# tayloreisman16/LTE-GNU-Radio-Code

Measured on AMD Instinct MI355X. Metric: IQ Msamples/s through RX FFT+equalize, 2048-pt/144-CP; %HBM roofline; 1/2/4/8 GPU, higher is better.
Workload: dtype f32; 1 GPU; 2048-pt FFT / 144-CP / Kd=1200 / 16-QAM, 4369 frames x 240 symbols (1,048,560 symbols), AWGN loopback; frames_per_gpu=4369, symbols_per_gpu=1048560, outputs=equalised symbols + packed bits, parallelism=frame-shard x1, sync_search=screened

## Files before the change

### lte-gnu-radio-code_amd/csrc/capi_internal.hpp

```cpp
#pragma once
#include <hip/hip_runtime.h>

#include <algorithm>
#include <cmath>
#include <complex>
#include <cstdarg>
#include <cstdio>
#include <cstdlib>
#include <cstring>
#include <initializer_list>
#include <new>
#include <string>
#include <vector>

#include "../../include/ofdm_mi355x.h"
#ifdef OFDM_EXPERIMENTS
#include "../../tools/experiments/ofdm_experiments.h"
#endif
#include "ofdm_launch.hpp"

using namespace ofdm;

#pragma GCC visibility push(hidden)
int fail(int code, const char* fmt, ...);
// ... 11 lines not shown
        if (e_ != hipSuccess) return fail(OFDM_ERR_HIP, "%s: %s", #expr, hipGetErrorString(e_));   \
    } while (0)

struct ofdm_rx {
    ofdm_rx_cfg cfg{};
    hipStream_t stream = nullptr;
    hipStream_t stream2 = nullptr;
    hipEvent_t ev_up = nullptr, ev_s1 = nullptr;
    RxDev dev{};
    cf* d_tw = nullptr;
    cf* d_zc = nullptr;
    int count = 0;
    int corr_obs = -1;
    double tsr[3] = {0, 0, 0};
    cf* d_in = nullptr;
    int64_t in_cap = 0;
    cf* d_edf = nullptr;
    cf* d_pack = nullptr;
    int* pin_tsr = nullptr;
    int* pin_tsr_dev = nullptr;
    static constexpr size_t PIN_IN_BYTES = size_t(1024) << 10, PIN_OUT_BYTES = size_t(256) << 10;
    cf* pin_in = nullptr;
    cf* pin_in_dev = nullptr;
    cf* pin_out = nullptr;
    cf* pin_out_dev = nullptr;
    int* s_tsr = nullptr;
    cf* s_H = nullptr;
    cf* s_htime = nullptr;
    cf* s_esf = nullptr;
    cf* s_eqg = nullptr;
    cf* s_gain = nullptr;
    cf* s_ysc = nullptr;
    float* d_trial_m = nullptr;
    int* d_trial_d = nullptr;
    static constexpr int TRIAL_CAP = 1024;
    double* d_partial = nullptr;
    int64_t cap_frames = 0;
    int* f_tsr = nullptr;
    cf* f_H = nullptr;
    cf* f_gain = nullptr;
    cf* f_htime = nullptr;
    int win_pre = 0, win_post = 0;
    float* f_tail = nullptr;
    int64_t tail_frames = -1;
    int avg_n = 0;
    float* f_spread = nullptr;
    int64_t spread_frames = -1;
    cf* a_part_d = nullptr;
    cf* a_part_a0 = nullptr;
    float* a_part_q = nullptr;
    int* a_part_n = nullptr;
    int64_t cap_avg_frames = 0, cap_avg_items = 0;
    double* f_seg_partial = nullptr;
    int64_t cap_seg_partial = 0;
    int n_pilots = 0;
    int* p_idx = nullptr;
    float* p_k = nullptr;
    uint16_t* p_src = nullptr;
    cf pilot_conj = cf{1.f, 0.f};
    float p_kbar = 0.f, p_inv_skk = 0.f;
    cf* f_usum = nullptr;
    int64_t cap_usum = 0;
    int64_t last_frames = 0;
    double* c_part_e = nullptr;
    long long* c_part_n = nullptr;
    int64_t cap_csi_items = 0;
    float2* c_tab = nullptr;
    float* c_a = nullptr;
    int64_t cap_csi_tab = 0;
    float2* m_tab = nullptr;
    int64_t cap_mrc_tab = 0;
    double* m_sigma2 = nullptr;
    int64_t cap_mrc_units = 0;
    float* t_ws = nullptr;
    int64_t cap_turbo = 0;
    uint8_t* tb_ws = nullptr;
    int64_t cap_tb = 0;
    int max_trials = 0;
    int scan_block = 0;
    cf* d_scan_g = nullptr;
    int* d_seg_state = nullptr;
    unsigned* d_work = nullptr;
    bool use_queue = true;
    bool seg_armed = false;
    int variant = 0;
    unsigned* d_stamps = nullptr;
    bool profiling = false;
    static constexpr int PROF_RING = 32;
    hipEvent_t ev[3 * PROF_RING] = {};
    int64_t prof_calls = 0;
};

struct ofdm_fo {
    ofdm_fo_cfg cfg{};
    hipStream_t stream = nullptr;
    RxDev dev{};
    cf* d_tw = nullptr;
    cf* d_zc = nullptr;
    cf* d_rot = nullptr;
    int count = 0;
    int cor_obs = -1;
    int dmax_tmp_ind = -1;
    double tsr[OFDM_FO_MAX_SYNC][3] = {};
    cf* d_in = nullptr;
    int64_t in_cap = 0;
    int* t_tsr = nullptr;
    cf* t_H = nullptr;
    cf* t_htime = nullptr;
    cf* t_esf = nullptr;
    cf* t_gain = nullptr;
    cf* t_edf = nullptr;
    cf* d_code = nullptr;
    cf* t_edfd = nullptr;
    int n_spread = 0;
    cf* s_eqg = nullptr;
    cf* s_ysc = nullptr;
    float* d_trial_m = nullptr;
    int* d_trial_d = nullptr;
    static constexpr int TRIAL_WIN = 256;
    int64_t cap_frames = 0;
    int64_t cap_table = 0;
    float* b_tm = nullptr;
    int* b_td = nullptr;
    int* b_tsr = nullptr;
    int* b_fo = nullptr;
    cf* b_gain = nullptr;
    cf* b_edf = nullptr;
};

struct ofdm_trk {
    ofdm_trk_cfg cfg{};
    hipStream_t stream = nullptr;
    RxDev dev{};
    cf* d_tw = nullptr;
    cf* d_zc = nullptr;
    cf* d_in = nullptr;
    int64_t in_cap = 0;
    int64_t n_in = 0;
    int* t_tsr = nullptr;
    cf* t_H = nullptr;
    cf* t_imp = nullptr;
    cf* t_esf = nullptr;
    cf* t_gain = nullptr;
    cf* t_edf = nullptr;
    cf* s_ysc = nullptr;
    float* d_trial_m = nullptr;
    int* d_trial_d = nullptr;
    static constexpr int TRIAL_CAP = 4096;
};

struct ofdm_tx {
    ofdm_tx_cfg cfg{};
    hipStream_t stream = nullptr;
    TxDev dev{};
    cf* d_tw = nullptr;
    cf* d_zc = nullptr;
    cf* d_sync_time = nullptr;
    int* d_pilots = nullptr;
    int n_pilots = 0;
    cf pilot_value = cf{1.f, 0.f};
    uint8_t* tb_ws = nullptr;
    int64_t cap_tb = 0;
};

namespace {

// ... 203 lines not shown
```

### lte-gnu-radio-code_amd/csrc/capi_rx.hip

```cpp
#include "capi_internal.hpp"

namespace {
constexpr int SEG_STATE_0[2] = {0x7fffffff, 0};
}

extern "C" {

int ofdm_rx_destroy(ofdm_rx* h) {
    if (!h) return OFDM_OK;
    (void)hipSetDevice(h->cfg.device);
    if (h->pin_tsr) (void)hipHostFree(h->pin_tsr);
    if (h->pin_in) (void)hipHostFree(h->pin_in);
    if (h->pin_out) (void)hipHostFree(h->pin_out);
    free_dev(&h->tb_ws, &h->d_pack, &h->d_tw, &h->d_zc, &h->d_in, &h->d_edf, &h->s_tsr, &h->s_H, &h->s_htime, &h->s_esf, &h->s_eqg, &h->s_gain,
             &h->s_ysc, &h->d_trial_m, &h->d_trial_d, &h->d_partial, &h->f_tsr, &h->f_H, &h->f_gain, &h->f_htime, &h->d_scan_g,
             &h->d_seg_state, &h->d_work, &h->f_seg_partial, &h->p_idx, &h->p_k, &h->p_src, &h->f_usum, &h->t_ws, &h->c_part_e,
             &h->c_part_n, &h->c_tab, &h->c_a, &h->m_tab, &h->m_sigma2, &h->f_tail, &h->f_spread, &h->a_part_d, &h->a_part_a0, &h->a_part_q, &h->a_part_n);
    for (hipEvent_t e : h->ev)
        if (e) (void)hipEventDestroy(e);
    if (h->ev_up) (void)hipEventDestroy(h->ev_up);
    if (h->ev_s1) (void)hipEventDestroy(h->ev_s1);
    if (h->stream2) (void)hipStreamDestroy(h->stream2);
    if (h->stream) (void)hipStreamDestroy(h->stream);
    delete h;
// ... 41 lines not shown
    h->d_stamps = static_cast<unsigned*>(d_stamps);
    return OFDM_OK;
}
#endif

int ofdm_rx_set_sync_search(ofdm_rx* h, int32_t exhaustive) {
    if (!h) return fail(OFDM_ERR_INVALID, "null handle");
    h->scan_block = exhaustive ? 0 : rx_sync_scan_block(h->dev);
    if (h->scan_block > 0 && !h->d_scan_g) h->scan_block = 0;
    return h->scan_block > 0 ? 1 : 0;
}

int ofdm_rx_set_max_trials(ofdm_rx* h, int32_t max_trials) {
    if (!h || max_trials < 0) return fail(OFDM_ERR_INVALID, "bad argument");
    h->max_trials = max_trials;
    return OFDM_OK;
}

int ofdm_rx_create(const ofdm_rx_cfg* c, ofdm_rx** out) {
    if (!c || !out) return fail(OFDM_ERR_INVALID, "ofdm_rx_create: null argument");
    *out = nullptr;
    if (int bad = check_nfft(c->nfft)) return bad;
    if (c->cp_len < 0 || c->cp_len >= c->nfft) return fail(OFDM_ERR_INVALID, "cp_len=%d out of range", c->cp_len);
    if (int bad = check_bins(c->nfft, c->num_synch_bins, c->num_data_bins)) return bad;
    if (int bad = check_pattern(c->synch_S, c->synch_D, c->num_ofdm_symb)) return bad;
    if (c->modulation != 1 && c->modulation != 2 && c->modulation != 4 && c->modulation != 6)
        return fail(OFDM_ERR_INVALID, "modulation must be 1, 2, 4 or 6 bits per symbol");
    if (c->compat == OFDM_COMPAT_RXOFDM && c->cp_len < 2)
        return fail(OFDM_ERR_INVALID, "gr-RXOFDM search stride is cp_len-1: cp_len must be >= 2");
    if (c->compat != OFDM_COMPAT_UTSA && c->compat != OFDM_COMPAT_RXOFDM) return fail(OFDM_ERR_INVALID, "bad compat");

    HIP_TRY(hipSetDevice(c->device));
    ofdm_rx* h = new (std::nothrow) ofdm_rx();
    if (!h) return fail(OFDM_ERR_NOMEM, "out of host memory");
    h->cfg = *c;
    const int N = c->nfft, Ks = c->num_synch_bins, Kd = c->num_data_bins, S = c->synch_S;
    const int MM = S * Ks;
    RxDev& d = h->dev;
    const int root = fill_rxdev(*c, d);

    int rc = OFDM_OK;
    hipError_t e = hipStreamCreateWithFlags(&h->stream, hipStreamNonBlocking);
    if (e != hipSuccess) {
        rc = fail(OFDM_ERR_HIP, "hipStreamCreate: %s", hipGetErrorString(e));
    }
    if (rc == OFDM_OK && (hipStreamCreateWithFlags(&h->stream2, hipStreamNonBlocking) != hipSuccess ||
                          hipEventCreateWithFlags(&h->ev_up, hipEventDisableTiming) != hipSuccess ||
                          hipEventCreateWithFlags(&h->ev_s1, hipEventDisableTiming) != hipSuccess))
        rc = fail(OFDM_ERR_HIP, "second stream / events of the stream block");
    auto zc = make_zc(MM, root, c->compat == OFDM_COMPAT_UTSA ? MM : Ks);
    const size_t rows = size_t(c->num_ofdm_symb);
    if (rc == OFDM_OK) rc = upload_rx_tables(d, &h->d_tw, &h->d_zc, zc);
    if (rc == OFDM_OK) rc = alloc_zeroed(&h->d_edf, rows * Kd);
    if (rc == OFDM_OK) rc = dev_alloc(&h->d_pack, rows * Kd);
    if (rc == OFDM_OK && (hipHostMalloc(reinterpret_cast<void**>(&h->pin_tsr), 4 * sizeof(int), hipHostMallocMapped) != hipSuccess ||
                          hipHostMalloc(reinterpret_cast<void**>(&h->pin_in), ofdm_rx::PIN_IN_BYTES, hipHostMallocMapped) != hipSuccess ||
                          hipHostMalloc(reinterpret_cast<void**>(&h->pin_out), ofdm_rx::PIN_OUT_BYTES, hipHostMallocMapped) != hipSuccess ||
                          hipHostGetDevicePointer(reinterpret_cast<void**>(&h->pin_tsr_dev), h->pin_tsr, 0) != hipSuccess ||
                          hipHostGetDevicePointer(reinterpret_cast<void**>(&h->pin_in_dev), h->pin_in, 0) != hipSuccess ||
                          hipHostGetDevicePointer(reinterpret_cast<void**>(&h->pin_out_dev), h->pin_out, 0) != hipSuccess))
        rc = fail(OFDM_ERR_NOMEM, "pinned host allocation failed");
    if (rc == OFDM_OK) rc = alloc_zeroed(&h->s_tsr, 4);
    if (rc == OFDM_OK) rc = alloc_zeroed(&h->s_H, size_t(2) * N);
    if (rc == OFDM_OK) rc = alloc_zeroed(&h->s_htime, size_t(2) * N);
    if (rc == OFDM_OK) rc = alloc_zeroed(&h->s_esf, size_t(2) * MM);
    if (rc == OFDM_OK) rc = alloc_zeroed(&h->s_eqg, size_t(Ks));
    if (rc == OFDM_OK) rc = alloc_zeroed(&h->s_gain, size_t(Kd));
    if (rc == OFDM_OK) rc = dev_alloc(&h->s_ysc, size_t(MM));
    if (rc == OFDM_OK) rc = dev_alloc(&h->d_trial_m, size_t(ofdm_rx::TRIAL_CAP));
    if (rc == OFDM_OK) rc = dev_alloc(&h->d_trial_d, size_t(ofdm_rx::TRIAL_CAP));
    if (rc == OFDM_OK) rc = dev_alloc(&h->d_partial, size_t(DEMAP_PARTIALS));
    if (rc == OFDM_OK) rc = alloc_zeroed(&h->d_work, 2, "work queue init failed");
    h->scan_block = rx_sync_scan_block(d);
    if (rc == OFDM_OK && h->scan_block > 0) {
        rc = upload(&h->d_scan_g, make_scan_table(N, Ks, zc), "scan table upload failed");
        if (rc == OFDM_OK) rc = upload(&h->d_seg_state, SEG_STATE_0, 2, "segment state upload failed");
        h->seg_armed = rc == OFDM_OK;
    }
    if (rc != OFDM_OK) return create_failed(h, rc, ofdm_rx_destroy);
#ifdef OFDM_EXPERIMENTS
    if (const char* ev = std::getenv("OFDM_EXP_VARIANT")) h->variant = std::atoi(ev);
#endif
    if (const char* q = std::getenv("OFDM_MI355X_DEMOD_QUEUE")) h->use_queue = std::atoi(q) != 0;
    *out = h;
    return OFDM_OK;
}

int ofdm_rx_reserve(ofdm_rx* h, int64_t n_frames) {
    if (!h || n_frames < 0) return fail(OFDM_ERR_INVALID, "ofdm_rx_reserve: bad argument");
    if (n_frames <= h->cap_frames) return OFDM_OK;
    h->last_frames = 0;
    h->tail_frames = -1;
    h->spread_frames = -1;
    return regrow(h, {{&h->cap_frames, n_frames}}, ws_buf(&h->f_tsr, size_t(n_frames) * 4),
                  ws_buf(&h->f_H, size_t(n_frames) * h->dev.nfft), ws_buf(&h->f_gain, size_t(n_frames) * h->dev.Kd),
                  ws_buf(&h->f_htime, size_t(n_frames) * h->dev.nfft), ws_buf(&h->f_tail, size_t(n_frames)),
                  ws_buf(&h->f_spread, size_t(n_frames)));
}

int64_t ofdm_rx_demod_frames(ofdm_rx* h, const float* d_iq, int64_t n_frames, int64_t frame_stride,
                             int64_t frame_len, float* d_eq, uint8_t* d_bits, int32_t bits_mode, int32_t* d_tsr,
                             void* stream) {
    if (!h || !d_iq || n_frames < 0 || frame_len < 0 || frame_stride < frame_len)
        return fail(OFDM_ERR_INVALID, "ofdm_rx_demod_frames: bad argument");
    const RxDev& d = h->dev;
    const int SD = d.S + d.D;
    const int64_t n_unique = frame_len / d.L;
    const int64_t n_pat = n_unique / SD;
    const int64_t n_dsym = n_pat * d.D;
    const char* bad = demod_bad_args(d, n_frames, n_dsym, d_bits, bits_mode);
    if (*bad) return fail(OFDM_ERR_INVALID, "%s", bad);
    if (n_frames == 0) return n_dsym;
    HIP_TRY(hipSetDevice(h->cfg.device));
    if (n_frames > h->cap_frames) {
        int rc = ofdm_rx_reserve(h, n_frames);
        if (rc != OFDM_OK) return rc;
    }
    hipStream_t s = pick_stream(h, stream);

    SyncArgs sa{};
    sa.iq = reinterpret_cast<const cf*>(d_iq);
    sa.frame_stride = frame_stride;
    sa.frame_len = frame_len;
    sa.n_frames = int(n_frames);
    sa.mode = 0;
    sa.p_begin = 0;
    sa.p_count = h->max_trials;
    sa.force_accept = 0;
    sa.tsr = h->f_tsr;
    sa.H = h->f_H;
    sa.H_for_gain = nullptr;
    sa.gain = h->f_gain;
    sa.htime = nullptr;
    sa.scan_block = h->scan_block;
    sa.scan_g = h->d_scan_g;
#ifdef OFDM_EXPERIMENTS
    sa.stamps = h->d_stamps;
#endif
    hipEvent_t* pev = h->ev + 3 * (h->prof_calls % ofdm_rx::PROF_RING);
    if (h->profiling) HIP_TRY(hipEventRecord(pev[0], s));
    HIP_TRY(launch_rx_sync(d, sa, s));
    h->last_frames = n_frames;
    h->tail_frames = -1;
    h->spread_frames = -1;
    if (h->avg_n != 0) {
        const int rc = chan_average_in_place(h, sa.iq, n_frames, frame_stride, frame_len, s);
        if (rc != OFDM_OK) return rc;
    }
    if (h->win_post > 0) {
        ChanWinArgs wa{};
        wa.H_in = h->f_H;
        wa.tsr = h->f_tsr;
        wa.n_rows = n_frames;
        wa.pre = h->win_pre;
        wa.post = h->win_post;
        wa.H_out = h->f_H;
        wa.gain = h->f_gain;
        wa.tail = h->f_tail;
        HIP_TRY(launch_chan_window(d, wa, s));
        h->tail_frames = n_frames;
    }
    if (h->profiling) HIP_TRY(hipEventRecord(pev[1], s));

    if (n_dsym > 0 && (d_eq || d_bits)) {
        DemodArgs da{};
        da.iq = sa.iq;
        da.frame_stride = frame_stride;
        da.frame_len = frame_len;
        da.n_frames = int(n_frames);
        da.tsr = h->f_tsr;
        da.gain = h->f_gain;
        da.eq = reinterpret_cast<cf*>(d_eq);
        da.bits = d_bits;
        da.bits_mode = bits_mode;
        da.mod = d.bps;
        da.n_dsym = int(n_dsym);
        da.spc = 0;
        da.chunks_per_frame = 0;
        da.row_stride_pat = d.D;
        da.rows_per_frame = int(n_dsym);
        da.zero_skipped = 1;
        da.variant = h->variant;
        da.stamps = h->d_stamps;
        da.work = h->use_queue ? h->d_work : nullptr;
        HIP_TRY(launch_rx_demod(d, da, s));
    }
    if (h->profiling) {
        HIP_TRY(hipEventRecord(pev[2], s));
        h->prof_calls += 1;
    }
    if (d_tsr) HIP_TRY(hipMemcpyAsync(d_tsr, h->f_tsr, size_t(n_frames) * 4 * sizeof(int), hipMemcpyDeviceToDevice, s));
    return n_dsym;
}

int ofdm_rx_get_frame_state(ofdm_rx* h, int64_t frame, float* h_chan_freq, float* h_gain, float* h_chan_time) {
    if (!h || frame < 0 || frame >= h->cap_frames) return fail(OFDM_ERR_INVALID, "ofdm_rx_get_frame_state: bad frame");
    HIP_TRY(hipSetDevice(h->cfg.device));
    HIP_TRY(hipDeviceSynchronize());
    const int N = h->dev.nfft, Kd = h->dev.Kd;
    if (h_chan_freq) HIP_TRY(hipMemcpy(h_chan_freq, h->f_H + frame * N, size_t(N) * sizeof(cf), hipMemcpyDeviceToHost));
    if (h_gain) HIP_TRY(hipMemcpy(h_gain, h->f_gain + frame * Kd, size_t(Kd) * sizeof(cf), hipMemcpyDeviceToHost));
    if (h_chan_time) {
        HIP_TRY(launch_rx_chan_time(h->dev, h->f_H + frame * N, h->f_htime + frame * N, 1, h->stream));
        HIP_TRY(hipStreamSynchronize(h->stream));
        HIP_TRY(hipMemcpy(h_chan_time, h->f_htime + frame * N, size_t(N) * sizeof(cf), hipMemcpyDeviceToHost));
    }
    return OFDM_OK;
}

int ofdm_rx_get_state(ofdm_rx* h, int32_t row, float* h_chan_freq, float* h_chan_time, float* h_synch_freq,
                      float* h_eq_gain, float* h_data_freq) {
    if (!h || row < 0 || row > 1) return fail(OFDM_ERR_INVALID, "ofdm_rx_get_state: bad argument");
    HIP_TRY(hipSetDevice(h->cfg.device));
    HIP_TRY(hipStreamSynchronize(h->stream));
    const int N = h->dev.nfft, Kd = h->dev.Kd, Ks = h->dev.Ks, MM = h->dev.MM;
    if (h_chan_freq) HIP_TRY(hipMemcpy(h_chan_freq, h->s_H + size_t(row) * N, size_t(N) * sizeof(cf), hipMemcpyDeviceToHost));
    if (h_chan_time) HIP_TRY(hipMemcpy(h_chan_time, h->s_htime + size_t(row) * N, size_t(N) * sizeof(cf), hipMemcpyDeviceToHost));
    if (h_synch_freq) HIP_TRY(hipMemcpy(h_synch_freq, h->s_esf + size_t(row) * MM, size_t(MM) * sizeof(cf), hipMemcpyDeviceToHost));
    if (h_eq_gain) HIP_TRY(hipMemcpy(h_eq_gain, h->s_eqg, size_t(Ks) * sizeof(cf), hipMemcpyDeviceToHost));
    if (h_data_freq)
        HIP_TRY(hipMemcpy(h_data_freq, h->d_edf, size_t(h->cfg.num_ofdm_symb) * Kd * sizeof(cf), hipMemcpyDeviceToHost));
    return OFDM_OK;
}

}
namespace {
hipError_t upload_in(ofdm_rx* h, const float* h_in, int64_t from, int64_t to, hipStream_t s) {
    return hipMemcpyAsync(h->d_in + from, h_in + 2 * from, size_t(to - from) * sizeof(cf), hipMemcpyHostToDevice, s);
}

int deleted_rows(int rows, int SD) {
    int n_del = 0;
    for (int r = 3; r < rows; r += SD) ++n_del;
    return n_del;
}

SyncArgs final_args(const ofdm_rx* h, const cf* iq, int64_t n_in, int row) {
    const RxDev& d = h->dev;
    SyncArgs fa{};
    fa.iq = iq;
    fa.frame_stride = n_in;
    fa.frame_len = n_in;
    fa.n_frames = 1;
    fa.mode = 0;
    fa.tsr = h->s_tsr;
    fa.H = h->s_H + size_t(row) * d.nfft;
    fa.H_for_gain = (row == 0) ? nullptr : h->s_H;
    fa.gain = h->s_gain;
    fa.htime = h->s_htime + size_t(row) * d.nfft;
    fa.esf = h->s_esf + size_t(row) * d.MM;
    fa.eqg = h->s_eqg;
    fa.yscratch = h->s_ysc;
    return fa;
}

void add_segments(SyncArgs& fa, const ofdm_rx* h, int64_t p0, int64_t p_valid) {
    fa.p_begin = int(p0);
    fa.p_count = int(p_valid);
    fa.keep_on_miss = 1;
    fa.scan_block = h->scan_block;
    fa.scan_g = h->d_scan_g;
    fa.seg_len = h->scan_block;
    fa.n_seg = int((p_valid - p0 + fa.seg_len - 1) / fa.seg_len);
    fa.seg_state = h->d_seg_state;
}

DemodArgs loop_b_args(const ofdm_rx* h, const cf* iq, int64_t n_in, int64_t n_dsym) {
// ... 267 lines not shown
```

### lte-gnu-radio-code_amd/csrc/ofdm_launch.hpp

```cpp
#pragma once
#include <hip/hip_runtime.h>
#include <stdint.h>
#include <algorithm>
#include <vector>
#include "ofdm_device.hpp"

namespace ofdm {

template <class... Kernel>
inline hipError_t load_kernels(Kernel*... kernels) {
    hipFuncAttributes fa;
    hipError_t e = hipSuccess;
    ((e = e == hipSuccess ? hipFuncGetAttributes(&fa, reinterpret_cast<const void*>(kernels)) : e), ...);
    return e;
}

struct DemodArgs {
    const cf* iq;
    int64_t frame_stride;
    int64_t frame_len;
    int n_frames;
    const int* tsr;
    const cf* gain;
    cf* eq;
    uint8_t* bits;
    int bits_mode;
    int mod;
    int n_dsym;
    int spc;
    int chunks_per_frame;
    int row_stride_pat;
    int rows_per_frame;
    int zero_skipped;
    int variant;
    unsigned* stamps;
    const cf* rot;
    int host_guard;
    unsigned* work;
    int units_per_frame;
    const int* rot_idx;
};

struct SyncArgs {
    const cf* iq;
    int64_t frame_stride;
    int64_t frame_len;
    int n_frames;
    int mode;
    int p_begin;
    int p_count;
    int force_accept;
    int* tsr;
    cf* H;
    const cf* H_for_gain;
    cf* gain;
    cf* htime;
    cf* esf;
    cf* eqg;
    cf* yscratch;
    float* trial_m;
    int* trial_d;
    const cf* rot;
    int n_rot;
    int off_delta;
    int host_valid;
    int gain_lag_set;
    int gain_lag;
    int force_dhat_p1;
    int scan_block;
    const cf* scan_g;
    unsigned* stamps;
    int keep_on_miss;
    int* tsr_host;
    int n_seg;
    int seg_len;
    int* seg_state;
    int seg_base;
    int seg_launch;
    int seg_final;
};

struct FoDecideArgs {
    const float* trial_m;
    const int* trial_d;
    int n_frames;
    int n_rot;
    int p_count;
    int rows;
    int err_index;
    int* status;
    int* tsr_out;
    int* fo_idx;
    int* u_tsr;
};

constexpr int SYNC_STAGE_SEGS = 64;

struct DemapArgs {
    const cf* sym;
    int64_t n;
    int mod;
    uint8_t* hard;
    float* soft0;
    float* soft1;
    double* partial;
};
constexpr int DEMAP_PARTIALS = 256;

constexpr int SEG_SLICE = 2048;
inline int64_t seg_slices(int64_t seg_len) { return (seg_len + SEG_SLICE - 1) / SEG_SLICE; }
enum : int { SEG_OUT_SOFT0 = 1, SEG_OUT_SOFT1 = 2, SEG_OUT_LLR = 4 };
struct SegDemapArgs {
    const cf* sym;
    int64_t n_seg, seg_len, seg_stride;
    int64_t n_slices;
    int mod;
    float* soft0;
    float* soft1;
    float* llr;
    double* sigma;
    double* partial;
};

// ... 420 lines not shown
```

### lte-gnu-radio-code_amd/csrc/rx_demod.hpp

```cpp
#pragma once
#include <algorithm>
#include <atomic>
#include <cstdlib>
#include <type_traits>

#include "ofdm_launch.hpp"
#include "demap_hard.hpp"

#ifndef OFDM_NS_T128
#define OFDM_NS_T128 2
#endif
#ifndef OFDM_MINW_T128
#define OFDM_MINW_T128 3
#endif
#ifndef OFDM_FLAGS_T128
#define OFDM_FLAGS_T128 0u
#endif
#ifndef OFDM_FLAGS_T256
#define OFDM_FLAGS_T256 0u
#endif
#ifndef OFDM_LANE_TW
#define OFDM_LANE_TW 1
#endif
#ifndef OFDM_SCATTER_HOIST
// ... 79 lines not shown
    int* const qslot = reinterpret_cast<int*>(smem + DG::Q_OFF);
    int64_t chunk = blockIdx.x;
    if (a.work) {
        if (tid == 0) *qslot = int(atomicAdd(a.work, 1u));
        __syncthreads();
        chunk = *qslot;
    }
    for (; chunk < n_chunks;) {
    const int frame = int(chunk / a.chunks_per_frame);
    const int cidx = int(chunk % a.chunks_per_frame);
    const int trips = (a.n_dsym + NS - 1) / NS;
    const int ds0 = int(int64_t(cidx) * trips / a.chunks_per_frame) * NS;
    const int ds1 = min(int(int64_t(cidx + 1) * trips / a.chunks_per_frame) * NS, a.n_dsym);
    constexpr bool active = true;

    const int Kd = KD > 0 ? KD : rx.Kd, L = rx.L, S = rx.S, D = rx.D;
    const int tsr0 = a.tsr[frame * 4 + 0];
    const bool frame_on = (HG || UNITS) ? (a.tsr[frame * 4 + 3] != 0) : true;
    const int src_frame = UNITS ? frame / a.units_per_frame : frame;
    const cf* frame_iq = a.iq + int64_t(L2IN ? (blockIdx.x & 7) : src_frame) * a.frame_stride;
    const cf* rotp = (UNITS && ROT) ? a.rot + int64_t(max(a.rot_idx[src_frame], 0)) * N : a.rot;

    const cf* gain = a.gain + int64_t(frame) * Kd;
    cf* glds = smem + DG::G_OFF;
    const cf* gsrc = GLDS ? glds : gain;
    if constexpr (GLDS) {
        for (int i = 2 * tid; i < Kd; i += 2 * DG::WG) *reinterpret_cast<float4*>(glds + i) = *reinterpret_cast<const float4*>(gain + i);
    }
    float4 greg[GREG ? Q : 1][2];
    if constexpr (GREG) {
#pragma unroll
        for (int q = 0; q < Q; ++q)
#pragma unroll
            for (int hx = 0; hx < 2; ++hx) {
                const int idx = 4 * T * q + 256 * (t >> 6) + 128 * hx + 2 * (t & 63);
                greg[q][hx] = idx < Kd ? *reinterpret_cast<const float4*>(gain + idx) : float4{0.f, 0.f, 0.f, 0.f};
            }
    }

    const float sqrt_kd = sqrtf(float(Kd));
    const int n_iter = (ds1 - ds0 + NS - 1) / NS;
    struct Sym {
        bool valid, compute;
        int64_t start, orow;
    };
    auto sym_of = [&](int it) {
        Sym sy;
        const int itr = it;
        const int ds = ds0 + itr * NS + slot;
        sy.valid = active && it < n_iter && ds < ds1;
        const int p = ds / D, n_ = ds - p * D;
        const int64_t pat_ptr = int64_t(tsr0) + int64_t(S) * L * (int64_t(p) * (S + D) + 1);
        sy.compute = sy.valid && (HG ? frame_on : (pat_ptr + N - 1 <= a.frame_len)) && (!UNITS || frame_on);
        sy.start = pat_ptr + int64_t(L) * n_;
        sy.orow = int64_t(frame) * a.rows_per_frame + (p * a.row_stride_pat + n_);
        return sy;
    };
    cf v[P];
    auto load_sym = [&](const Sym& sy) {
        if (sy.compute && sy.start >= 0 && sy.start + N <= a.frame_len) {
            const cf* src = frame_iq + sy.start + t;
#pragma unroll
            for (int n0 = 0; n0 < P; ++n0) v[n0] = NTL ? __builtin_nontemporal_load(src + T * n0) : src[T * n0];
            if constexpr (ROT) {
#pragma unroll
                for (int n0 = 0; n0 < P; ++n0) v[n0] = cmul(v[n0], rotp[t + T * n0]);
            }
        } else {
            const int64_t before = -sy.start, left = a.frame_len - sy.start;
            const int lo = int(before < 0 ? 0 : (before < N ? before : N)), hi = int(left < 0 ? 0 : (left < N ? left : N));
            const bool any = sy.compute && hi > lo;
            int tq = t;
            asm volatile("" : "+v"(tq));
#pragma unroll
            for (int n0 = 0; n0 < P; ++n0) {
                const int e = tq + T * n0;
                const cf x = any ? frame_iq[sy.start + min(max(e, lo), hi - 1)] : cf{0.f, 0.f};
                v[n0] = (any && e >= lo && e < hi) ? x : cf{0.f, 0.f};
                if constexpr (ROT) v[n0] = cmul(v[n0], rotp[tq + T * n0]);
            }
        }
    };

    Sym cur = sym_of(0);
    if constexpr (PIPE) load_sym(cur);
    if constexpr (WL) wg_barrier();
    for (int it = 0; it < n_iter; ++it) {
        if constexpr (!PIPE) {
            cur = sym_of(it);
            load_sym(cur);
        }
        const bool sym_valid = cur.valid, compute = cur.compute;
        const int64_t orow = cur.orow;
        stamp(0);
        if constexpr (STAMP) asm volatile("s_waitcnt vmcnt(0)" ::: "memory");
        stamp(1);
        if constexpr (STAMP) {
            fft_pass0_store<N>(v, lds, tw, t);
            wg_barrier();
            stamp(2);
            if constexpr (PL::THREE) {
                fft_pass1_load<N>(v, lds, t);
                wg_barrier();
                fft_pass1_store<N>(v, lds, w1tab, t);
                wg_barrier();
            }
            stamp(3);
            fft_last_load<N>(v, lds, t);
            fft_last_dft<N>(v);
        } else {
            wg_fft<N, decltype(tw), WL>(v, lds, tw, w1tab, t);
        }
        slot_sync<WL>();

        int Kd_ = Kd;
#if !OFDM_SCATTER_HOIST
        asm volatile("" : "+s"(Kd_));
#endif
        const int hk = Kd_ >> 1;
        const int off_neg = hk - N, off_pos = hk - 1;
        float pse = 0.f;
#pragma unroll
        for (int j = 0; j < PL::C; ++j) {
#pragma unroll
            for (int kl = 0; kl < PL::RL; ++kl) {
#if OFDM_SCATTER_SKIP
                if constexpr (T >= 64) {
                    const int base = T * j + PL::NC * kl;
                    if (base > hk && base + T - 1 < N - hk) continue;
                }
#endif
                const int k = (t + T * j) + PL::NC * kl;
#if OFDM_SCATTER_SKIP
                if constexpr (T >= 64) {
                    const int base = T * j + PL::NC * kl;
                    const bool all_pos = base >= 1 && base + T - 1 <= hk, all_neg = base >= N - hk && hk < N / 2;
                    if (all_pos || all_neg) {
                        lds[k + (all_neg ? off_neg : off_pos)] = v[out_slot<N>(j, kl)];
                        if constexpr (PSE) pse += cnorm2(v[out_slot<N>(j, kl)]);
                        continue;
                    }
                }
#endif
                int i = k + ((k >= N - hk) ? off_neg : off_pos);
                if (j == 0 && kl == 0) i = (k == 0) ? N : i;
                lds[i] = v[out_slot<N>(j, kl)];
                if constexpr (PSE) pse += (unsigned(i) < unsigned(Kd_)) ? cnorm2(v[out_slot<N>(j, kl)]) : 0.f;
            }
        }
        if (Kd_ == N) {
#pragma unroll
            for (int j = 0; j < PL::C; ++j) {
#pragma unroll
                for (int kl = 0; kl < PL::RL; ++kl)
                    if ((t + T * j) + PL::NC * kl == N / 2) {
                        lds[N - 1] = v[out_slot<N>(j, kl)];
                        if constexpr (PSE) pse += cnorm2(v[out_slot<N>(j, kl)]);
                    }
            }
        }
        if constexpr (PSE) {
            pse = lanes_sum<T>(pse);
            if constexpr (T > 64) {
                if ((t & 63) == 0) red[t >> 6] = pse;
            }
        }
// ... 84 lines not shown
                                g = greg[q][hx];
                            else
                                g = *reinterpret_cast<const float4*>(g_lane + cofs);
                            const float4 av = *reinterpret_cast<const float4*>(l_lane + cofs);
                            cf z[2] = {cf{av.x, av.y} * scale, cf{av.z, av.w} * scale};
                            cmul2(z[0], cf{g.x, g.y}, z[1], cf{g.z, g.w});
                            if (eq_row) {
                                typedef float f4 __attribute__((ext_vector_type(4)));
                                const f4 ov = f4{z[0].x, z[0].y, z[1].x, z[1].y};
                                cf* const blk = eq_row + cofs;
#ifdef OFDM_EXPERIMENTS
                                constexpr unsigned SPOL = (FLAGS >> 12) & 3u;
                                if constexpr (SPOL == 1) {
                                    asm volatile("global_store_dwordx4 %0, %1, %2 sc1" ::"v"(eq_off), "v"(ov), "s"(blk) : "memory");
                                } else if constexpr (SPOL == 2) {
                                    asm volatile("global_store_dwordx4 %0, %1, %2 sc0 sc1" ::"v"(eq_off), "v"(ov), "s"(blk) : "memory");
                                } else if constexpr (SPOL == 3) {
                                    asm volatile("global_store_dwordx4 %0, %1, %2 sc0 sc1 nt" ::"v"(eq_off), "v"(ov), "s"(blk) : "memory");
                                } else
#endif
                                if constexpr (NT) {
                                    asm volatile("global_store_dwordx4 %0, %1, %2 nt" ::"v"(eq_off), "v"(ov), "s"(blk) : "memory");
                                } else {
                                    asm volatile("global_store_dwordx4 %0, %1, %2" ::"v"(eq_off), "v"(ov), "s"(blk) : "memory");
                                }
                            }
                            if constexpr (BMODE == 1) wp[hx] = pack2<MOD, ASMB>(z);
                            if constexpr (BMODE == 2) store_bits_pair_unpacked<MOD>(bits_row + cofs * MOD, unsigned(lane_e), z);
                        };
                        if (base + 128 <= Kd_) {
                            pair();
                        } else if (base < Kd_) {
                            if (base + 2 * lnm < Kd_) pair();
                        }
                    }
                    if constexpr (BMODE == 1) {
                        const bool odd = (ln & 1) != 0;
                        const unsigned recv = unsigned(__builtin_amdgcn_mov_dpp(int(odd ? wp[0] : wp[1]), 0xB1, 0xF, 0xF, false));
                        const unsigned w4 = odd ? ((recv << (2 * MOD)) | wp[1]) : ((wp[0] << (2 * MOD)) | recv);
                        const int ge = lane_e + (odd ? 126 : 0);
                        uint8_t* const brow = bits_row + (4 * T * q / 4) * (MOD / 2);
                        if (b0 + 256 <= Kd_) {
                            store_packed4<MOD>(brow, unsigned(ge), w4);
                        } else if (4 * T * q + ((KD > 0) ? opaque_lane(ge) : ge) < Kd_) {
                            store_packed4<MOD>(brow, unsigned(ge), w4);
                        }
                    }
                }
            }
        } else {
#pragma unroll
            for (int q = 0; q < Q; ++q) {
                const int idx = 4 * (t + T * q);
                if (idx < Kd_) {
                    const bool four = idx + 2 < Kd_;
                    const float4 g01 = *reinterpret_cast<const float4*>(gsrc + idx);
                    const float4 g23 = (GLDS || four) ? *reinterpret_cast<const float4*>(gsrc + idx + 2) : float4{0.f, 0.f, 0.f, 0.f};
                    const float4 a01 = *reinterpret_cast<const float4*>(lds + idx);
                    const float4 a23 = *reinterpret_cast<const float4*>(lds + idx + 2);
                    cf z[4] = {cf{a01.x, a01.y} * scale, cf{a01.z, a01.w} * scale, cf{a23.x, a23.y} * scale,
                               cf{a23.z, a23.w} * scale};
                    cmul3(z[0], cf{g01.x, g01.y}, z[1], cf{g01.z, g01.w}, z[2], cf{g23.x, g23.y});
                    z[3] = cmul(z[3], cf{g23.z, g23.w});
                    if (a.eq) {
                        float4* o = reinterpret_cast<float4*>(a.eq + orow * Kd_ + idx);
                        const float4 o0 = float4{z[0].x, z[0].y, z[1].x, z[1].y}, o1 = float4{z[2].x, z[2].y, z[3].x, z[3].y};
                        if constexpr (NT) {
                            typedef float f4 __attribute__((ext_vector_type(4)));
                            f4* on = reinterpret_cast<f4*>(o);
                            __builtin_nontemporal_store(f4{o0.x, o0.y, o0.z, o0.w}, on);
                            if (four) __builtin_nontemporal_store(f4{o1.x, o1.y, o1.z, o1.w}, on + 1);
                        } else {
                            o[0] = o0;
                            if (four) o[1] = o1;
                        }
                    }
                    if constexpr (BMODE != 0) store_bits<MOD, BMODE, ASMB>(a.bits, orow * Kd_ + idx, z, four ? 4 : 2);
                }
            }
        }
        stamp(6);
        slot_sync<WL>();
        stamp(7);
    }
    if (!a.work) break;
    __syncthreads();
    if (tid == 0) *qslot = int(atomicAdd(a.work, 1u));
    __syncthreads();
    chunk = *qslot;
    }
    if (a.work) {
        if (tid == 0 && atomicAdd(a.work + 1, 1u) == gridDim.x - 1) {
            atomicExch(a.work, 0u);
            atomicExch(a.work + 1, 0u);
        }
    }
    if constexpr (STAMP) {
        if ((tid & 63) == 0 && a.stamps) {
            unsigned* o = a.stamps + (int64_t(blockIdx.x) * (DG::WG / 64) + (tid >> 6)) * 8;
#pragma unroll
            for (int i = 0; i < 8; ++i) o[i] = acc[i];
        }
    }
}

template <int N, int KD>
hipError_t launch_rx_demod_batch(const RxDev& rx, DemodArgs a, unsigned grid, size_t lds, int bmode, hipStream_t s) {
    using DG = DemodGeom<N>;
    constexpr int MW = (Plan<N>::T == 128) ? OFDM_MINW_T128 : 3;
    constexpr unsigned FL = (Plan<N>::T == 128) ? OFDM_FLAGS_T128 : (Plan<N>::T == 256) ? OFDM_FLAGS_T256 : 0u;
#define OFDM_LD(M, B)                                                                                                        \
    do {                                                                                                                     \
        static std::atomic<int> announced{65536};                \
        if (int(lds) > announced.load(std::memory_order_relaxed)) {                                                          \
            hipError_t e = hipFuncSetAttribute(reinterpret_cast<const void*>(&rx_demod_kernel<N, M, B, MW, FL, KD>),         \
                                               hipFuncAttributeMaxDynamicSharedMemorySize, int(lds));                       \
            if (e != hipSuccess) return e;                                                                                   \
            announced.store(int(lds), std::memory_order_relaxed);                                                            \
        }                                                                                                                    \
        hipLaunchKernelGGL((rx_demod_kernel<N, M, B, MW, FL, KD>), dim3(grid), dim3(DG::WG), lds, s, rx, a);                 \
    } while (0)
    if (N < 1024) a.work = nullptr;
    if (a.work) {
        static int per_cu = 0, n_cu = 0;
        if (per_cu == 0) {
            int nb = 0, dev = 0;
            hipDeviceProp_t prop;
            if (hipOccupancyMaxActiveBlocksPerMultiprocessor(&nb, rx_demod_kernel<N, 4, 1, MW, FL, KD>, DG::WG, lds) != hipSuccess || nb < 1) nb = 2;
            n_cu = (hipGetDevice(&dev) == hipSuccess && hipGetDeviceProperties(&prop, dev) == hipSuccess && prop.multiProcessorCount > 0)
                       ? prop.multiProcessorCount : 256;
            per_cu = nb;
        }
        const int64_t resident = int64_t(per_cu) * n_cu;
        if (int64_t(grid) > 2 * resident)
            grid = unsigned(resident);
        else
            a.work = nullptr;
    }
#define OFDM_LD_MOD(B)                  \
    switch (a.mod) {                    \
        case 1: OFDM_LD(1, B); break;   \
        case 2: OFDM_LD(2, B); break;   \
        case 4: OFDM_LD(4, B); break;   \
        default: OFDM_LD(6, B); break;  \
    }
    if (bmode == 0) {
        OFDM_LD(2, 0);
    } else if (bmode == 1) {
        OFDM_LD_MOD(1)
    } else {
        OFDM_LD_MOD(2)
    }
#undef OFDM_LD_MOD
#undef OFDM_LD
    return hipGetLastError();
}

#define OFDM_EXTERN_DEMOD_KD(n) \
    extern template hipError_t launch_rx_demod_batch<n, DemodGeom<n>::KD_LTE>(const RxDev&, DemodArgs, unsigned, size_t, int, hipStream_t);
OFDM_EXTERN_DEMOD_KD(1024)
OFDM_EXTERN_DEMOD_KD(2048)
OFDM_EXTERN_DEMOD_KD(4096)
#undef OFDM_EXTERN_DEMOD_KD

template <int N>
hipError_t launch_rx_demod_n(const RxDev& rx, const DemodArgs& a_in, hipStream_t s) {
// ... 113 lines not shown
```

Baseline: 607,800 Msamples/s.

## Add fast demod path for fully in-bounds symbol chunks with per-wave specialization

Adds a specialized demodulation loop that runs when every symbol in a chunk lies within the frame and no flags or rotation apply. It drops per-sample bounds clamping, uses scalar (SGPR) base addresses with nontemporal loads and stores, and prefetches the next symbol after the FFT. It also instantiates a separate copy of the loop per wave index so the lane offsets are compile-time constants. The path is on by default and can be turned off with an environment variable. The costs are larger code size, more register pressure, and a second code path that has to stay consistent with the general one.

```diff
diff --git a/lte-gnu-radio-code_amd/csrc/capi_internal.hpp b/lte-gnu-radio-code_amd/csrc/capi_internal.hpp
--- a/lte-gnu-radio-code_amd/csrc/capi_internal.hpp
+++ b/lte-gnu-radio-code_amd/csrc/capi_internal.hpp
@@ -117,6 +117,7 @@
     int* d_seg_state = nullptr;
     unsigned* d_work = nullptr;
     bool use_queue = true;
+    bool demod_fast = true;
     bool seg_armed = false;
     int variant = 0;
     unsigned* d_stamps = nullptr;
diff --git a/lte-gnu-radio-code_amd/csrc/capi_rx.hip b/lte-gnu-radio-code_amd/csrc/capi_rx.hip
--- a/lte-gnu-radio-code_amd/csrc/capi_rx.hip
+++ b/lte-gnu-radio-code_amd/csrc/capi_rx.hip
@@ -147,6 +147,7 @@
     if (const char* ev = std::getenv("OFDM_EXP_VARIANT")) h->variant = std::atoi(ev);
 #endif
     if (const char* q = std::getenv("OFDM_MI355X_DEMOD_QUEUE")) h->use_queue = std::atoi(q) != 0;
+    if (const char* q = std::getenv("OFDM_MI355X_DEMOD_FAST")) h->demod_fast = std::atoi(q) != 0;
     *out = h;
     return OFDM_OK;
 }
@@ -248,6 +249,7 @@
         da.variant = h->variant;
         da.stamps = h->d_stamps;
         da.work = h->use_queue ? h->d_work : nullptr;
+        da.fast = h->demod_fast ? 1 : 0;
         HIP_TRY(launch_rx_demod(d, da, s));
     }
     if (h->profiling) {
diff --git a/lte-gnu-radio-code_amd/csrc/ofdm_launch.hpp b/lte-gnu-radio-code_amd/csrc/ofdm_launch.hpp
--- a/lte-gnu-radio-code_amd/csrc/ofdm_launch.hpp
+++ b/lte-gnu-radio-code_amd/csrc/ofdm_launch.hpp
@@ -39,6 +39,7 @@
     unsigned* work;
     int units_per_frame;
     const int* rot_idx;
+    int fast;
 };
 
 struct SyncArgs {
diff --git a/lte-gnu-radio-code_amd/csrc/rx_demod.hpp b/lte-gnu-radio-code_amd/csrc/rx_demod.hpp
--- a/lte-gnu-radio-code_amd/csrc/rx_demod.hpp
+++ b/lte-gnu-radio-code_amd/csrc/rx_demod.hpp
@@ -185,6 +185,198 @@
         }
     };
 
+    auto scatter_bins = [&](int Kd_) __attribute__((always_inline)) {
+        const int hk = Kd_ >> 1;
+        const int off_neg = hk - N, off_pos = hk - 1;
+        float pse = 0.f;
+#pragma unroll
+        for (int j = 0; j < PL::C; ++j) {
+#pragma unroll
+            for (int kl = 0; kl < PL::RL; ++kl) {
+#if OFDM_SCATTER_SKIP
+                if constexpr (T >= 64) {
+                    const int base = T * j + PL::NC * kl;
+                    if (base > hk && base + T - 1 < N - hk) continue;
+                }
+#endif
+                const int k = (t + T * j) + PL::NC * kl;
+#if OFDM_SCATTER_SKIP
+                if constexpr (T >= 64) {
+                    const int base = T * j + PL::NC * kl;
+                    const bool all_pos = base >= 1 && base + T - 1 <= hk, all_neg = base >= N - hk && hk < N / 2;
+                    if (all_pos || all_neg) {
+                        lds[k + (all_neg ? off_neg : off_pos)] = v[out_slot<N>(j, kl)];
+                        if constexpr (PSE) pse += cnorm2(v[out_slot<N>(j, kl)]);
+                        continue;
+                    }
+                }
+#endif
+                int i = k + ((k >= N - hk) ? off_neg : off_pos);
+                if (j == 0 && kl == 0) i = (k == 0) ? N : i;
+                lds[i] = v[out_slot<N>(j, kl)];
+                if constexpr (PSE) pse += (unsigned(i) < unsigned(Kd_)) ? cnorm2(v[out_slot<N>(j, kl)]) : 0.f;
+            }
+        }
+        if (Kd_ == N) {
+#pragma unroll
+            for (int j = 0; j < PL::C; ++j) {
+#pragma unroll
+                for (int kl = 0; kl < PL::RL; ++kl)
+                    if ((t + T * j) + PL::NC * kl == N / 2) {
+                        lds[N - 1] = v[out_slot<N>(j, kl)];
+                        if constexpr (PSE) pse += cnorm2(v[out_slot<N>(j, kl)]);
+                    }
+            }
+        }
+        if constexpr (PSE) {
+            pse = lanes_sum<T>(pse);
+            if constexpr (T > 64) {
+                if ((t & 63) == 0) red[t >> 6] = pse;
+            }
+        }
+        return pse;
+    };
+
+    constexpr bool FAST = FLAGS == 0 && DENSE && KD > 0 && T >= 128;
+    bool fast_done = false;
+    if constexpr (FAST) {
+        const int dl = ds1 - 1, pl = dl / D;
+        const int64_t last_start = int64_t(tsr0) + int64_t(S) * L * (int64_t(pl) * (S + D) + 1) + int64_t(L) * (dl - pl * D);
+        const bool plain = a.fast && n_iter > 0 && n_iter * NS == ds1 - ds0 && tsr0 >= 0 && last_start + N <= a.frame_len &&
+                           a.eq != nullptr && (a.bits != nullptr) == (BMODE != 0);
+        if (plain) {
+            const int ln = t & 63;
+            const int lnm = opaque_lane(ln);
+            const int frame_u = __builtin_amdgcn_readfirstlane(frame), ds0_u = __builtin_amdgcn_readfirstlane(ds0),
+                      tsr0_u = __builtin_amdgcn_readfirstlane(tsr0), trips_u = __builtin_amdgcn_readfirstlane(n_iter);
+            const cf* const iq_u = a.iq + int64_t(frame_u) * a.frame_stride;
+            auto plain_sym = [&](int it, int64_t& start, int64_t& row0) __attribute__((always_inline)) {
+                const int ds = ds0_u + it * NS + slot;
+                const int p = __builtin_amdgcn_readfirstlane(ds / D), n_ = ds - p * D;
+                start = int64_t(tsr0_u) + int64_t(S) * L * (int64_t(p) * (S + D) + 1) + int64_t(L) * n_;
+                row0 = (int64_t(frame_u) * a.rows_per_frame + (p * a.row_stride_pat + n_)) * KD;
+            };
+            auto sbase = [](auto* ptr) __attribute__((always_inline)) {
+                typedef __attribute__((address_space(1))) std::remove_pointer_t<decltype(ptr)> G;
+                uint64_t u = reinterpret_cast<uint64_t>(ptr);
+                asm("" : "+s"(u));
+                return reinterpret_cast<G*>(u);
+            };
+            auto load_plain = [&](int64_t start) __attribute__((always_inline)) {
+                constexpr int G = (T * int(sizeof(cf)) >= 4096) ? 1 : 4096 / (T * int(sizeof(cf)));
+#pragma unroll
+                for (int g = 0; g < P; g += G) {
+                    const auto* const src = sbase(iq_u + start + T * g);
+#pragma unroll
+                    for (int j = 0; j < G && g + j < P; ++j) v[g + j] = __builtin_nontemporal_load(src + (unsigned(t) + unsigned(T * j)));
+                }
+            };
+            auto trip = [&](auto wtag, auto last, int it) __attribute__((always_inline)) {
+                constexpr int W = decltype(wtag)::value;
+                constexpr bool LAST = decltype(last)::value;
+                int64_t start, row0, next_start, next_row0;
+                plain_sym(it, start, row0);
+                wg_fft<N, decltype(tw), WL>(v, lds, tw, w1tab, t);
+                slot_sync<WL>();
+                const float pse = scatter_bins(KD);
+                slot_sync<WL>();
+                if constexpr (!LAST) {
+                    plain_sym(it + 1, next_start, next_row0);
+                    load_plain(next_start);
+                }
+                float psum = 0.f;
+                if constexpr (T > 64) {
+#pragma unroll
+                    for (int w = 0; w < T / 64; ++w) psum += red[w];
+                } else {
+                    psum = pse;
+                }
+                const float scale = sqrt_kd * __builtin_amdgcn_rsqf(psum);
+
+                const int lane_e = 256 * W + 2 * opaque_lane(ln);
+                const cf* const l_lane = lds + lane_e;
+                const cf* const g_lane = gsrc + lane_e;
+                typedef float f4 __attribute__((ext_vector_type(4)));
+                uint8_t* const bits_row = (BMODE == 0) ? nullptr : (BMODE == 1) ? a.bits + ((row0 * MOD) >> 3) : a.bits + row0 * MOD;
+#pragma unroll
+                for (int q = 0; q < Q; ++q) {
+                    const int b0 = 4 * T * q + 256 * W;
+                    if (b0 >= KD) continue;
+                    unsigned wp[2] = {0u, 0u};
+                    auto* const eq_q = sbase(a.eq + row0 + 4 * T * q);
+                    float4 g[2], av[2];
+                    auto read = [&](int hx) __attribute__((always_inline)) {
+                        g[hx] = *reinterpret_cast<const float4*>(g_lane + (4 * T * q + 128 * hx));
+                        av[hx] = *reinterpret_cast<const float4*>(l_lane + (4 * T * q + 128 * hx));
+                    };
+                    auto finish = [&](int hx) __attribute__((always_inline)) {
+                        const int cofs = 4 * T * q + 128 * hx;
+                        cf z[2] = {cf{av[hx].x, av[hx].y} * scale, cf{av[hx].z, av[hx].w} * scale};
+                        cmul2(z[0], cf{g[hx].x, g[hx].y}, z[1], cf{g[hx].z, g[hx].w});
+                        const f4 ov = f4{z[0].x, z[0].y, z[1].x, z[1].y};
+                        typedef __attribute__((address_space(1))) char GC;
+                        __builtin_nontemporal_store(ov, reinterpret_cast<__attribute__((address_space(1))) f4*>(
+                                                            reinterpret_cast<GC*>(eq_q) + unsigned(lane_e + 128 * hx) * unsigned(sizeof(cf))));
+                        if constexpr (BMODE == 1) wp[hx] = pack2<MOD, ASMB>(z);
+                        if constexpr (BMODE == 2) store_bits_pair_unpacked<MOD>(bits_row + cofs * MOD, unsigned(lane_e), z);
+                    };
+#pragma unroll
+                    for (int hx = 0; hx < 2; ++hx)
+                        if (b0 + 128 * hx + 128 <= KD) read(hx);
+#pragma unroll
+                    for (int hx = 0; hx < 2; ++hx) {
+                        const int base = b0 + 128 * hx;
+                        if (base + 128 <= KD) {
+                            finish(hx);
+                        } else if (base < KD) {
+                            if (base + 2 * lnm < KD) {
+                                read(hx);
+                                finish(hx);
+                            }
+                        }
+                    }
+                    if constexpr (BMODE == 1) {
+                        const bool odd = (ln & 1) != 0;
+                        const unsigned recv = unsigned(__builtin_amdgcn_mov_dpp(int(odd ? wp[0] : wp[1]), 0xB1, 0xF, 0xF, false));
+                        const unsigned w4 = odd ? ((recv << (2 * MOD)) | wp[1]) : ((wp[0] << (2 * MOD)) | recv);
+                        const int ge = lane_e + (odd ? 126 : 0);
+                        uint8_t* const brow = bits_row + (4 * T * q / 4) * (MOD / 2);
+                        if (b0 + 256 <= KD) {
+                            store_packed4<MOD>(brow, unsigned(ge), w4);
+                        } else if (4 * T * q + opaque_lane(ge) < KD) {
+                            store_packed4<MOD>(brow, unsigned(ge), w4);
+                        }
+                    }
+                }
+                slot_sync<WL>();
+            };
+            auto run = [&](auto wtag) __attribute__((always_inline)) {
+                int64_t start, row0;
+                plain_sym(0, start, row0);
+                load_plain(start);
+                if constexpr (WL) wg_barrier();
+#pragma unroll
+                for (int n0 = 0; n0 < P; ++n0) asm volatile("" : "+v"(v[n0]));
+                for (int it = 0; it + 1 < trips_u; ++it) trip(wtag, std::false_type{}, it);
+                trip(wtag, std::true_type{}, trips_u - 1);
+            };
+            const int wv = __builtin_amdgcn_readfirstlane(t >> 6);
+            if constexpr (T <= 64) {
+                run(std::integral_constant<int, 0>{});
+            } else if constexpr (T == 128) {
+                if (wv == 0) run(std::integral_constant<int, 0>{});
+                else run(std::integral_constant<int, 1>{});
+            } else {
+                static_assert(T == 256, "one copy of the fast loop per wave of a slot");
+                if (wv == 0) run(std::integral_constant<int, 0>{});
+                else if (wv == 1) run(std::integral_constant<int, 1>{});
+                else if (wv == 2) run(std::integral_constant<int, 2>{});
+                else run(std::integral_constant<int, 3>{});
+            }
+            fast_done = true;
+        }
+    }
+    if (!fast_done) {
     Sym cur = sym_of(0);
     if constexpr (PIPE) load_sym(cur);
     if constexpr (WL) wg_barrier();
@@ -435,6 +627,7 @@
         stamp(6);
         slot_sync<WL>();
         stamp(7);
+    }
     }
     if (!a.work) break;
     __syncthreads();
```

Measured after the change: 609,700 Msamples/s, median of 6. Within noise of the previous version (+0.3%).
